# oxfordcontrol/Clarabel.rs

Hardware: NVIDIA H100
Metric: ipm_iterations_per_sec (higher is better)
Workload: dtype f64

## Files before the change

### clarabel.rs_b200/csrc/ldl.cu

```cuda
#include <cuda_runtime.h>
#include <dlfcn.h>

#include <cmath>
#include <cstdio>
#include <cstring>
#include <algorithm>
#include <thread>
#include <vector>

#include "../../include/clarabel_b200.h"
#include "ldl_device.h"
#include "symbolic.h"
#include "vec.cuh"

namespace cb {

std::atomic<unsigned long long> g_launches{0};

typedef struct ncclComm* cb_ncclComm_t;
typedef struct { char internal[128]; } cb_ncclUniqueId;
struct NcclApi {
  void* lib = nullptr;
  int (*GetUniqueId)(cb_ncclUniqueId*) = nullptr;
  int (*CommInitRank)(cb_ncclComm_t*, int, cb_ncclUniqueId, int) = nullptr;
  int (*AllGather)(const void*, void*, size_t, int, cb_ncclComm_t, cudaStream_t) = nullptr;
  int (*CommDestroy)(cb_ncclComm_t) = nullptr;
  const char* (*GetErrorString)(int) = nullptr;
};
static NcclApi* nccl_api(const char* libpath) {
  static NcclApi api;
  static bool tried = false;
  if (api.lib) return &api;
  if (tried && !libpath) return nullptr;
  tried = true;
  void* h = dlopen(libpath && *libpath ? libpath : "libnccl.so.2", RTLD_NOW | RTLD_GLOBAL);
  if (!h) { std::fprintf(stderr, "[clarabel_b200] dlopen(%s) failed: %s\n", libpath ? libpath : "libnccl.so.2", dlerror()); return nullptr; }
  api.GetUniqueId = (int (*)(cb_ncclUniqueId*))dlsym(h, "ncclGetUniqueId");
  api.CommInitRank = (int (*)(cb_ncclComm_t*, int, cb_ncclUniqueId, int))dlsym(h, "ncclCommInitRank");
  api.AllGather = (int (*)(const void*, void*, size_t, int, cb_ncclComm_t, cudaStream_t))dlsym(h, "ncclAllGather");
  api.CommDestroy = (int (*)(cb_ncclComm_t))dlsym(h, "ncclCommDestroy");
  api.GetErrorString = (const char* (*)(int))dlsym(h, "ncclGetErrorString");
  if (!api.GetUniqueId || !api.CommInitRank || !api.AllGather || !api.CommDestroy) return nullptr;
  api.lib = h;
  return &api;
}



template <int NT>
__device__ __forceinline__ void pivot_inverse(double* A, int lda, int ns) {
  for (int j = threadIdx.x; j < ns; j += NT) {
    for (int i = j + 1; i < ns; i++) {
      double a0 = A[(long long)j * lda + i], a1 = 0.0;
      int k = j + 1;
      for (; k + 1 < i; k += 2) {
        a0 += A[(long long)k * lda + i] * A[(long long)k * lda + j];
        a1 += A[(long long)(k + 1) * lda + i] * A[(long long)(k + 1) * lda + j];
      }
      if (k < i) a0 += A[(long long)k * lda + i] * A[(long long)k * lda + j];
      A[(long long)i * lda + j] = -(a0 + a1);
    }
  }
}
template <int NT>
__device__ __forceinline__ void pivot_inverse_place(double* A, int lda, int ns) {
  for (int idx = threadIdx.x; idx < ns * ns; idx += NT) {
    const int j = idx / ns, i = idx - j * ns;
    if (i > j) {
      A[(long long)j * lda + i] = A[(long long)i * lda + j];
      A[(long long)i * lda + j] = 0.0;
    }
  }
}

template <int NT>
__global__ void __launch_bounds__(NT) k_factor_level(LDLDev d, int task_base, int smem_cap) {
  extern __shared__ double sm[];
  __shared__ double sD[CB_MAX_PANEL];
  __shared__ double sInv[CB_MAX_PANEL];
  const int tid = threadIdx.x;
  const int lane = tid & 31, warp = tid >> 5, nwarp = NT >> 5;
  const int s = d.level_tasks[task_base + blockIdx.x];
  const int f = d.sn_first[s];
  const int ns = d.sn_first[s + 1] - f;
  const long long rp = d.sn_rowptr[s];
  const int nr = (int)(d.sn_rowptr[s + 1] - rp);
  const int ld = ns + nr;
  double* __restrict__ P = d.L + d.panel_off[s];
  double* __restrict__ U = d.U + d.upd_off[s];
  const long long psz = (long long)ld * ns;
  const bool use_sm = psz <= (long long)smem_cap;
  double* W = use_sm ? sm : P;

  for (long long i = tid; i < psz; i += NT) W[i] = 0.0;
  __syncthreads();
  for (long long e = d.asm_ptr[s] + tid; e < d.asm_ptr[s + 1]; e += NT)
    W[d.asm_dst[e]] = d.vals[d.asm_src[e]];

  int c_reg = 0, c_pos = 0, c_zero = 0, c_nonf = 0;
  for (int j = 0; j < ns; j++) {
    __syncthreads();
    const double* __restrict__ cj = W + (long long)j * ld;
    double dj = cj[j];
    bool reg = false;
    if (d.reg_enable) {
      const double sg = (double)d.dsigns[f + j];
      if (dj * sg < d.reg_eps) { dj = d.reg_delta * sg; reg = true; }
    }
    const double inv = 1.0 / dj;
    if (tid == 0) {
      c_reg += reg ? 1 : 0;
      c_pos += dj > 0.0 ? 1 : 0;
      if (dj == 0.0) c_zero = 1;
      if (!isfinite(inv)) c_nonf = 1;
      d.D[f + j] = dj;
      d.Dinv[f + j] = inv;
      sD[j] = dj;
      sInv[j] = inv;
    }
    for (int k = j + 1 + warp; k < ns; k += nwarp) {
      const double wk = cj[k] * inv;
      double* __restrict__ ck = W + (long long)k * ld;
      for (int i = k + lane; i < ld; i += 32) ck[i] -= cj[i] * wk;
    }
  }
  __syncthreads();
  for (int j = warp; j < ns; j += nwarp) {
    double* __restrict__ cj = W + (long long)j * ld;
    const double inv = sInv[j];
    if (lane == 0) cj[j] = sD[j];
    for (int i = j + 1 + lane; i < ld; i += 32) cj[i] *= inv;
  }
  if (tid == 0) {
    if (c_reg) atomicAdd(&d.status[ST_REGCOUNT], c_reg);
    if (c_pos) atomicAdd(&d.status[ST_POSINERTIA], c_pos);
    if (c_zero) atomicExch(&d.status[ST_ZEROPIV], 1);
    if (c_nonf) atomicExch(&d.status[ST_NONFINITE], 1);
  }
  __syncthreads();

  {
    int it = 0;
    for (int b0 = 0; b0 < nr; b0 += 4)
      for (int a0 = b0; a0 < nr; a0 += 32, it++) {
        if (it % nwarp != warp) continue;
        const int a = a0 + lane;
        const bool on = a < nr;
        const int nb = min(4, nr - b0);
        double acc[4] = {0.0, 0.0, 0.0, 0.0};
        const double* __restrict__ ck = W + ns;
        for (int k = 0; k < ns; k++, ck += ld) {
          const double la = on ? ck[a] : 0.0, dk = sD[k];
#pragma unroll
          for (int c = 0; c < 4; c++) acc[c] += la * (ck[b0 + min(c, nb - 1)] * dk);
        }
#pragma unroll
        for (int c = 0; c < 4; c++)
          if (on && b0 + c < nr && a >= b0 + c) U[(long long)(b0 + c) * nr + a] = 0.0 - acc[c];
      }
  }
  if (ns > CB_SOLVE_SMALL_NS) {
    pivot_inverse<NT>(W, ld, ns);
    __syncthreads();
    pivot_inverse_place<NT>(W, ld, ns);
  }
  if (use_sm) {
    __syncthreads();
    for (long long i = tid; i < psz; i += NT) P[i] = W[i];
  }
}

#define LEAF1_NT 256
#define LEAF1_MAXLD 128
static_assert(LEAF1_MAXLD > CB_BIG_NR, "a level-0 column must fit the per-warp buffer");
__global__ void __launch_bounds__(LEAF1_NT) k_factor_leaf1(LDLDev d, int task_base, int count) {
  __shared__ double s_col[LEAF1_NT / 32][LEAF1_MAXLD];
  __shared__ int s_pos, s_reg;
  const int lane = threadIdx.x & 31, warp = threadIdx.x >> 5;
  const int i = blockIdx.x * (LEAF1_NT / 32) + warp;
  if (threadIdx.x == 0) { s_pos = 0; s_reg = 0; }
  __syncthreads();
  if (i < count) {
    double* col = s_col[warp];
    const int s = d.level_tasks[task_base + i];
    const int f = d.sn_first[s];
    const long long rp = d.sn_rowptr[s];
    const int nr = (int)(d.sn_rowptr[s + 1] - rp);
    const int ld = 1 + nr;
    double* __restrict__ P = d.L + d.panel_off[s];
    double* __restrict__ U = d.U + d.upd_off[s];
    for (int a = lane; a < ld; a += 32) col[a] = 0.0;
    __syncwarp();
    for (long long e = d.asm_ptr[s] + lane; e < d.asm_ptr[s + 1]; e += 32) col[d.asm_dst[e]] = d.vals[d.asm_src[e]];
    __syncwarp();
    double dj = col[0];
    bool reg = false;
    if (d.reg_enable) {
      const double sg = (double)d.dsigns[f];
      if (dj * sg < d.reg_eps) { dj = d.reg_delta * sg; reg = true; }
    }
    const double inv = 1.0 / dj;
    if (lane == 0) {
      if (dj == 0.0) atomicExch(&d.status[ST_ZEROPIV], 1);
      if (!isfinite(inv)) atomicExch(&d.status[ST_NONFINITE], 1);
      if (dj > 0.0) atomicAdd(&s_pos, 1);
      if (reg) atomicAdd(&s_reg, 1);
      d.D[f] = dj;
      d.Dinv[f] = inv;
    }
    __syncwarp();
    for (int a = lane; a < ld; a += 32) {
      const double v = a == 0 ? dj : col[a] * inv;
      col[a] = v;
      P[a] = v;
    }
    __syncwarp();
    for (int idx = lane; idx < nr * nr; idx += 32) {
      const int b = idx / nr, a = idx - b * nr;
      if (a >= b) {
        const double t = col[1 + b] * dj;
        double acc = 0.0;
        acc += col[1 + a] * t;
        U[idx] = 0.0 - acc;
      }
    }
  }
  __syncthreads();
  if (threadIdx.x == 0) {
    if (s_pos) atomicAdd(&d.status[ST_POSINERTIA], s_pos);
    if (s_reg) atomicAdd(&d.status[ST_REGCOUNT], s_reg);
  }
}

__global__ void k_permute_in(int n, const int* __restrict__ perm, const double* __restrict__ b,
                             double* __restrict__ xp) {
  int k = blockIdx.x * blockDim.x + threadIdx.x;
  if (k < n) xp[k] = b[perm[k]];
}

__device__ __forceinline__ unsigned long long df_gtime() {
#ifdef CB_EMU
  return 0;
#else
  unsigned long long t;
  asm volatile("mov.u64 %0, %%globaltimer;" : "=l"(t));
  return t;
#endif
}
__device__ __forceinline__ void df_wait_zero(volatile int* p) {
  unsigned ns = 20;
  while (*p > 0) { __nanosleep(ns); if (ns < 640) ns <<= 1; }
}
__device__ __forceinline__ void df_wait_set(volatile int* p) {
  unsigned ns = 20;
  while (*p == 0) { __nanosleep(ns); if (ns < 640) ns <<= 1; }
}

#include "ldl_solve.cuh"

#define DF_NT 256
#define DF_SMEM_DOUBLES (CB_PB_MAXNS * CB_PB_LD + 2 * CB_PB_MAXNS + CB_PB_MAXNS * 128)

__device__ __forceinline__ double ldcg_d(const double* p) { return __ldcg(p); }

template <class Map>
__device__ __forceinline__ void df_apply_sorted(double* base, const double* __restrict__ U,
                                                const int* __restrict__ esrc, const int* __restrict__ edst,
                                                int e0, int e1, Map map) {
  const int cnt = e1 - e0;
  if (cnt <= 0) return;
  const int per = (cnt + DF_NT - 1) / DF_NT;
  int b = e0 + threadIdx.x * per, e = min(e1, b + per);
  if (b >= e1) return;
  if (b > e0) { while (b < e1 && edst[b] == edst[b - 1]) b++; }
  if (e < e1) { while (e < e1 && edst[e] == edst[e - 1]) e++; }
  int i = b;
  while (i < e) {
    const int dd = edst[i];
    double acc = 0.0;
    while (i < e && edst[i] == dd) { acc += __ldcg(U + esrc[i]); i++; }
    const long long t = map(dd);
    if (t >= 0) base[t] += acc;
  }
}

__shared__ int df_cur_qi;
#define DF_STAMP(q, slot) do { if ((q).trace && threadIdx.x == 0) (q).trace[10 * (size_t)df_cur_qi + (slot)] = df_gtime(); } while (0)
__device__ __forceinline__ void df_front_complete(const DFFactor& q, int s) {
  const int p = q.parent[s];
  if (p >= 0) atomicSub(q.pend + p, 1);
}

__device__ void dff_small(const LDLDev& d, int s, double* sm, int* s_flag) {
  __shared__ double s_inv;
  const int tid = threadIdx.x, lane = tid & 31, warp = tid >> 5, nwarp = DF_NT >> 5;
  const int f = d.sn_first[s];
  const int ns = d.sn_first[s + 1] - f;
  const long long rp = d.sn_rowptr[s];
  const int nr = (int)(d.sn_rowptr[s + 1] - rp);
  const int ld = ns + nr;
  double* P = d.L + d.panel_off[s];
  double* U = d.U + d.upd_off[s];
  const long long psz = (long long)ld * ns;
  double* sD = sm;
  double* Wsm = sm + CB_MAX_PANEL;
  const bool use_sm = psz <= (long long)(DF_SMEM_DOUBLES - CB_MAX_PANEL);
  double* W = use_sm ? Wsm : P;
  (void)s_flag;
  for (long long i = tid; i < psz; i += DF_NT) W[i] = 0.0;
  for (int b = warp; b < nr; b += nwarp)
    for (int a = b + lane; a < nr; a += 32) U[(long long)b * nr + a] = 0.0;
  __syncthreads();
  for (long long e = d.asm_ptr[s] + tid; e < d.asm_ptr[s + 1]; e += DF_NT) W[d.asm_dst[e]] = d.vals[d.asm_src[e]];
  __syncthreads();
  for (long long ci = d.child_ptr[s]; ci < d.child_ptr[s + 1]; ci++) {
    const int c = d.child_list[ci];
    const long long crp = d.sn_rowptr[c];
    const int nrc = (int)(d.sn_rowptr[c + 1] - crp);
    const double* Uc = d.U + d.upd_off[c];
    const int* __restrict__ relc = d.rel + crp;
    for (int b = warp; b < nrc; b += nwarp) {
      const int rb = relc[b];
      for (int a = b + lane; a < nrc; a += 32) {
        const int ra = relc[a];
        const double v = __ldcg(Uc + (long long)b * nrc + a);
        if (rb < ns) W[(long long)rb * ld + ra] += v;
        else U[(long long)(rb - ns) * nr + (ra - ns)] += v;
      }
    }
    __syncthreads();
  }
  int c_reg = 0, c_pos = 0, c_zero = 0, c_nonf = 0;
  for (int j = 0; j < ns; j++) {
    if (tid == 0) {
      double dj = W[(long long)j * ld + j];
      if (d.reg_enable) {
        const double sg = (double)d.dsigns[f + j];
        if (dj * sg < d.reg_eps) { dj = d.reg_delta * sg; c_reg++; }
      }
      if (dj == 0.0) c_zero = 1;
      if (dj > 0.0) c_pos++;
      const double inv = 1.0 / dj;
      if (!isfinite(inv)) c_nonf = 1;
      d.D[f + j] = dj;
      d.Dinv[f + j] = inv;
      W[(long long)j * ld + j] = dj;
      s_inv = inv;
      sD[j] = dj;
    }
    __syncthreads();
    const double inv = s_inv;
    const double* cj = W + (long long)j * ld;
    for (int k = j + 1 + warp; k < ns; k += nwarp) {
      const double wk = cj[k] * inv;
      double* ck = W + (long long)k * ld;
      for (int i = k + lane; i < ld; i += 32) ck[i] -= cj[i] * wk;
    }
    __syncthreads();
    double* cjw = W + (long long)j * ld;
    for (int i = j + 1 + tid; i < ld; i += DF_NT) cjw[i] *= inv;
  }
  __syncthreads();
  if (tid == 0) {
    if (c_reg) atomicAdd(&d.status[ST_REGCOUNT], c_reg);
    if (c_pos) atomicAdd(&d.status[ST_POSINERTIA], c_pos);
    if (c_zero) atomicExch(&d.status[ST_ZEROPIV], 1);
    if (c_nonf) atomicExch(&d.status[ST_NONFINITE], 1);
  }
  for (int b = warp; b < nr; b += nwarp)
    for (int a = b + lane; a < nr; a += 32) {
      double acc = 0.0;
      for (int k = 0; k < ns; k++) {
        const double* ck = W + (long long)k * ld + ns;
        acc += ck[a] * (ck[b] * sD[k]);
      }
      U[(long long)b * nr + a] -= acc;
    }
  if (ns > CB_SOLVE_SMALL_NS) {
    pivot_inverse<DF_NT>(W, ld, ns);
    __syncthreads();
    pivot_inverse_place<DF_NT>(W, ld, ns);
    __syncthreads();
  }
  if (use_sm) for (long long i = tid; i < psz; i += DF_NT) P[i] = W[i];
}

#define DF_DCAP 32
#define DF_REC_INTS ((int)(sizeof(DFChildRec) / sizeof(int)))
#define DF_REC_INT(r, field) (reinterpret_cast<const int*>(r)[offsetof(DFChildRec, field) / sizeof(int)])

template <int NH>
__device__ __forceinline__ void df_add_child(const LDLDev& d, const DFChildRec& ch, double* dst, int rowoff,
                                             int rstride, int coloff, int cstride) {
  const int lane = threadIdx.x & 31, warp = threadIdx.x >> 5;
  const int* __restrict__ relc = d.rel + ch.relp;
  const double* Uc = d.U + ch.uoff;
  __syncwarp();
  if (ch.contig == 3) {
    const int r0 = ch.ra0 - rowoff - ch.a0, c0 = ch.rb0 - coloff - ch.b0;
    const int bfirst = ch.b0 + ((warp - (c0 + ch.b0)) & 7);
    const int a1 = ch.a1, b1 = ch.b1;
    for (int ab = ch.a0; ab < a1; ab += 32 * NH) {
      double v[8][NH];
#pragma unroll
      for (int c = 0; c < 8; c++) {
        const int b = bfirst + 8 * c;
#pragma unroll
        for (int h = 0; h < NH; h++) {
          const int a = ab + lane + 32 * h;
          v[c][h] = (b < b1 && a < a1 && a >= b) ? __ldcg(Uc + (long long)b * ch.nrc + a) : 0.0;
        }
      }
#pragma unroll
      for (int c = 0; c < 8; c++) {
        const int b = bfirst + 8 * c;
#pragma unroll
        for (int h = 0; h < NH; h++) {
          const int a = ab + lane + 32 * h;
          if (b < b1 && a < a1 && a >= b) dst[(r0 + a) * rstride + (c0 + b) * cstride] += v[c][h];
        }
      }
    }
    __syncwarp();
    return;
  }
  const int bl = ch.b0 + lane, bh = bl + 32;
  const int dc0 = bl < ch.b1 ? relc[bl] - coloff : -1;
  const int dc1 = bh < ch.b1 ? relc[bh] - coloff : -1;
  unsigned m0 = __ballot_sync(0xffffffffu, dc0 >= 0 && (dc0 & 7) == warp);
  unsigned m1 = __ballot_sync(0xffffffffu, dc1 >= 0 && (dc1 & 7) == warp);
  const int cnt0 = __popc(m0), cnt = cnt0 + __popc(m1);
  const int oc = lane >> 2, ar = lane & 3;
  int pos = -1;
  if (oc < cnt) {
    unsigned m = oc < cnt0 ? m0 : m1;
    const int skip = oc < cnt0 ? oc : oc - cnt0;
    for (int k = 0; k < skip; k++) m &= m - 1;
    pos = __ffs(m) - 1 + (oc < cnt0 ? 0 : 32);
  }
  const int srcl = pos < 0 ? 0 : (pos & 31);
  const int x0 = __shfl_sync(0xffffffffu, dc0, srcl), x1 = __shfl_sync(0xffffffffu, dc1, srcl);
  if (pos >= 0) {
    const int dcc = (pos < 32 ? x0 : x1) * cstride;
    const int b = ch.b0 + pos;
    const double* ucol = Uc + (long long)b * ch.nrc;
    const int a1 = ch.a1;
    for (int a = max(ch.a0, b) + ar; a < a1; a += 32) {
      double v[8];
      int r[8];
#pragma unroll
      for (int u = 0; u < 8; u++) {
        const int aa = a + 4 * u;
        const bool ok = aa < a1;
        v[u] = ok ? __ldcg(ucol + aa) : 0.0;
        r[u] = ok ? relc[aa] : rowoff;
      }
#pragma unroll
      for (int u = 0; u < 8; u++)
        if (a + 4 * u < a1) dst[(r[u] - rowoff) * rstride + dcc] += v[u];
    }
  }
  __syncwarp();
}

#define DF_ENT_FAST (2 * DF_NT)
struct DFEnt { int dd[2]; double v[2]; };
__device__ __forceinline__ void df_ent_issue(const double* __restrict__ U, const int* __restrict__ esrc,
                                             const int* __restrict__ edst, int e0, int e1, DFEnt& pe) {
  const int cnt = e1 - e0;
  pe.dd[0] = pe.dd[1] = -1;
  pe.v[0] = pe.v[1] = 0.0;
  if (cnt > DF_ENT_FAST) return;
  int src[2] = {0, 0};
#pragma unroll
  for (int u = 0; u < 2; u++) {
    const int i = threadIdx.x + u * DF_NT;
    if (i < cnt) { pe.dd[u] = edst[e0 + i]; src[u] = esrc[e0 + i]; }
  }
#pragma unroll
  for (int u = 0; u < 2; u++)
    if (threadIdx.x + u * DF_NT < cnt) pe.v[u] = __ldcg(U + src[u]);
}
template <class Map>
__device__ __forceinline__ void df_ent_apply(double* base, const double* __restrict__ U, const int* __restrict__ esrc,
                                             const int* __restrict__ edst, int e0, int e1, const DFEnt& pe,
                                             int* s_ed, double* s_ev, Map map) {
  const int cnt = e1 - e0;
  if (cnt <= 0) return;
  if (cnt > DF_ENT_FAST) { df_apply_sorted(base, U, esrc, edst, e0, e1, map); return; }
#pragma unroll
  for (int u = 0; u < 2; u++) {
    const int i = threadIdx.x + u * DF_NT;
    if (i < cnt) { s_ed[i] = pe.dd[u]; s_ev[i] = pe.v[u]; }
  }
  __syncthreads();
#pragma unroll
  for (int u = 0; u < 2; u++) {
    int i = threadIdx.x + u * DF_NT;
    if (i < cnt) {
      const int dd = pe.dd[u];
      if (i == 0 || s_ed[i - 1] != dd) {
        double acc = 0.0;
        while (i < cnt && s_ed[i] == dd) { acc += s_ev[i]; i++; }
        const long long t = map(dd);
        if (t >= 0) base[t] += acc;
      }
    }
  }
}

template <class Put>
__device__ __forceinline__ void df_scatter_asm(const LDLDev& d, int s, Put put) {
  const long long e0 = d.asm_ptr[s], e1 = d.asm_ptr[s + 1];
  for (long long e = e0 + threadIdx.x; e < e1; e += 4 * DF_NT) {
    long long dst[4];
    int src[4];
    double v[4];
#pragma unroll
    for (int u = 0; u < 4; u++) {
      const long long ee = e + (long long)u * DF_NT;
      const bool ok = ee < e1;
      dst[u] = ok ? (long long)d.asm_dst[ee] : -1;
      src[u] = ok ? d.asm_src[ee] : 0;
    }
#pragma unroll
    for (int u = 0; u < 4; u++) v[u] = dst[u] >= 0 ? d.vals[src[u]] : 0.0;
#pragma unroll
    for (int u = 0; u < 4; u++) if (dst[u] >= 0) put(dst[u], v[u]);
  }
}

template <class F>
__device__ __forceinline__ void df_children(const DFFactor& q, int d0, int d1, int* s_desc, F f) {
  for (int base = d0; base < d1; base += DF_DCAP) {
    const int cnt = min(DF_DCAP, d1 - base);
    const int* src = reinterpret_cast<const int*>(q.recs);
    for (int i = threadIdx.x; i < cnt * DF_REC_INTS; i += DF_NT) s_desc[i] = src[(size_t)base * DF_REC_INTS + i];
// ... 230 lines not shown
  DF_STAMP(q, 6);
#ifdef CB_EMU
  const int tx = tid & 15, ty = tid >> 4;
#define OWN_R(i) (tx + 16 * (i))
#define OWN_C(j) (ty + 16 * (j))
#else
  const int lk = tid & 3, lr = (tid & 31) >> 2, r0w = ((tid >> 5) & 1) * 32, c0w = (tid >> 6) * 16;
#define OWN_R(i) (r0w + 8 * (i) + lr)
#define OWN_C(j) (c0w + 8 * ((j) >> 1) + 2 * lk + ((j) & 1))
#endif
  double creg[4][4];
#pragma unroll
  for (int i = 0; i < 4; i++)
#pragma unroll
    for (int j = 0; j < 4; j++) creg[i][j] = 0.0;
  const int ndense = tk.ndense;
  for (int kd = 0; kd < ndense; kd++) {
    const DFChildRec* rec = q.recs + (size_t)(tk.d0 + kd);
    const long long uoff = rec->uoff;
    const int nrc = DF_REC_INT(rec, nrc), a0 = DF_REC_INT(rec, a0), a1 = DF_REC_INT(rec, a1), b0 = DF_REC_INT(rec, b0), b1 = DF_REC_INT(rec, b1);
    const int ra = a0 - (DF_REC_INT(rec, ra0) - (ns + i0)), rb = b0 - (DF_REC_INT(rec, rb0) - (ns + j0));
    const double* Uc = d.U + uoff;
    double v[4][4];
#pragma unroll
    for (int j = 0; j < 4; j++) {
      const int b = OWN_C(j) + rb;
#pragma unroll
      for (int i = 0; i < 4; i++) {
        const int a = OWN_R(i) + ra;
        v[i][j] = (a >= a0 && a < a1 && b >= b0 && b < b1 && a >= b) ? __ldcg(Uc + (long long)b * nrc + a) : 0.0;
      }
    }
#pragma unroll
    for (int i = 0; i < 4; i++)
#pragma unroll
      for (int j = 0; j < 4; j++) creg[i][j] += v[i][j];
  }
  const bool use_sc = (tk.d1 - tk.d0 > ndense) || (tk.e1 > tk.e0);
  if (use_sc) {
    for (int idx = tid; idx < TS * (TS + 1); idx += DF_NT) sC[idx] = 0.0;
    __syncthreads();
    DF_STAMP(q, 7);
    df_children(q, tk.d0 + ndense, tk.d1, s_desc, [&](const DFChildRec& ch) { df_add_child<2>(d, ch, sC, ns + i0, TS + 1, ns + j0, 1); });
    DF_STAMP(q, 8);
    df_ent_apply(sC, d.U, d.sc_tile_src, d.sc_tile_dst, tk.e0, tk.e1, pe, s_ed, s_ev, [&](int dd) -> long long { return dd; });
  }
#ifndef CB_EMU
  asm volatile("cp.async.wait_group 0;" ::: "memory");
#endif
  __syncthreads();
  for (int idx = tid; idx < ns * TS; idx += DF_NT) sBt[idx] *= sD[idx >> 6];
#ifndef CB_EMU
  {
    const int ns4 = (ns + 3) & ~3;
    for (int idx = ns * TS + tid; idx < ns4 * TS; idx += DF_NT) { sAt[idx] = 0.0; sBt[idx] = 0.0; }
  }
#endif
  __syncthreads();
  DF_STAMP(q, 4);
#ifdef CB_EMU
  double acc[4][4];
#pragma unroll
  for (int i = 0; i < 4; i++)
#pragma unroll
    for (int j = 0; j < 4; j++) acc[i][j] = 0.0;
#pragma unroll 4
  for (int k = 0; k < ns; k++) {
    double a[4], b[4];
#pragma unroll
    for (int i = 0; i < 4; i++) { a[i] = sAt[k * TS + tx + 16 * i]; b[i] = sBt[k * TS + ty + 16 * i]; }
#pragma unroll
    for (int i = 0; i < 4; i++)
#pragma unroll
      for (int j = 0; j < 4; j++) acc[i][j] += a[i] * b[j];
  }
#else
  double c2[4][2][2];
  {
#pragma unroll
    for (int i = 0; i < 4; i++)
#pragma unroll
      for (int j = 0; j < 2; j++) { c2[i][j][0] = 0.0; c2[i][j][1] = 0.0; }
    const int ns4 = (ns + 3) & ~3;
#pragma unroll 2
    for (int k = 0; k < ns4; k += 4) {
      double a[4], b[2];
#pragma unroll
      for (int i = 0; i < 4; i++) a[i] = sAt[(k + lk) * TS + r0w + 8 * i + lr];
#pragma unroll
      for (int j = 0; j < 2; j++) b[j] = sBt[(k + lk) * TS + c0w + 8 * j + lr];
#pragma unroll
      for (int i = 0; i < 4; i++)
#pragma unroll
        for (int j = 0; j < 2; j++)
          asm volatile("mma.sync.aligned.m8n8k4.row.col.f64.f64.f64.f64 {%0,%1}, {%2}, {%3}, {%0,%1};"
                       : "+d"(c2[i][j][0]), "+d"(c2[i][j][1]) : "d"(a[i]), "d"(b[j]));
    }
  }
#endif
  DF_STAMP(q, 5);
#pragma unroll
  for (int i = 0; i < 4; i++) {
    const int rr = OWN_R(i);
#pragma unroll
    for (int j = 0; j < 4; j++) {
      const int cc = OWN_C(j);
#ifdef CB_EMU
      const double prod = acc[i][j];
#else
      const double prod = c2[i][j >> 1][j & 1];
#endif
      if (rr < ni && cc < nj && (i0 + rr >= j0 + cc))
        U[(long long)(j0 + cc) * nr + (i0 + rr)] = (use_sc ? creg[i][j] + sC[rr * (TS + 1) + cc] : creg[i][j]) - prod;
    }
  }
#undef OWN_R
#undef OWN_C
}

__global__ void __launch_bounds__(DF_NT, 2) k_factor_df(LDLDev d, DFFactor q) {
  extern __shared__ __align__(16) double dfsm[];
  __shared__ __align__(16) int s_desc[DF_DCAP * DF_REC_INTS];
  __shared__ __align__(16) int s_task[16];
  __shared__ int s_ed[DF_ENT_FAST];
  __shared__ double s_ev[DF_ENT_FAST];
  __shared__ int s_last;
  const int tid = threadIdx.x;
  if (tid == 0) df_cur_qi = -1;
  for (;;) {
    __syncthreads();
    if (tid == 0) {
      if (q.trace && df_cur_qi >= 0) q.trace[10 * (size_t)df_cur_qi + 2] = df_gtime();
      const int qi = atomicAdd(q.qhead, 1);
      df_cur_qi = qi < q.ntask ? qi : -1;
      if (q.trace && df_cur_qi >= 0) {
        unsigned smid = 0;
#ifndef CB_EMU
        asm volatile("mov.u32 %0, %%smid;" : "=r"(smid));
#endif
        q.trace[10 * (size_t)qi] = df_gtime();
        q.trace[10 * (size_t)qi + 3] = smid;
      }
    }
    __syncthreads();
    const int qi = df_cur_qi;
    if (qi < 0) break;
    if (tid < 4) reinterpret_cast<int4*>(s_task)[tid] = q.tasks[4 * (size_t)qi + tid];
    __syncthreads();
    const DFTask& tk = *reinterpret_cast<const DFTask*>(s_task);
    const int kind = tk.kind, s = tk.s;
    if (kind == 0) {
      if (tid == 0) { df_wait_zero(q.pend + s); __threadfence(); if (q.trace) q.trace[10 * (size_t)qi + 1] = df_gtime(); }
      __syncthreads();
      dff_small(d, s, dfsm, nullptr);
      __syncthreads();
      if (tid == 0) { __threadfence(); df_front_complete(q, s); }
    } else if (kind == 1) {
      if (tid == 0) { df_wait_zero(q.pend + s); __threadfence(); if (q.trace) q.trace[10 * (size_t)qi + 1] = df_gtime(); }
      __syncthreads();
      dff_diag(d, q, tk, dfsm, s_desc, s_ed, s_ev);
      __syncthreads();
      if (tid == 0) { __threadfence(); atomicExch(q.diag_done + s, 1); }
    } else if (kind == 2) {
      if (tid == 0) { df_wait_zero(q.pend + s); __threadfence(); if (q.trace) q.trace[10 * (size_t)qi + 1] = df_gtime(); }
      __syncthreads();
      dff_rows(d, q, tk, dfsm, s_desc, s_ed, s_ev);
      __syncthreads();
      if (tid == 0) { __threadfence(); s_last = atomicSub(q.rows_left + s, 1) == 1; }
      __syncthreads();
      if (s_last && tk.ns > CB_SOLVE_SMALL_NS) dff_rows_invert(d, tk, dfsm);
    } else {
      if (tid == 0) { df_wait_zero(q.rows_left + s); __threadfence(); if (q.trace) q.trace[10 * (size_t)qi + 1] = df_gtime(); }
      __syncthreads();
      dff_tile(d, q, tk, dfsm, s_desc, s_ed, s_ev);
      __syncthreads();
      if (tid == 0) {
        __threadfence();
        if (atomicSub(q.tiles_left + s, 1) == 1) df_front_complete(q, s);
      }
    }
  }
}

__global__ void k_update_values(double* __restrict__ vals, const int* __restrict__ idx,
                                const double* __restrict__ v, long long len) {
  long long i = (long long)blockIdx.x * blockDim.x + threadIdx.x;
  if (i < len) vals[idx[i]] = v[i];
}
__global__ void k_scale_values(double* __restrict__ vals, const int* __restrict__ idx, double s,
                               long long len) {
  long long i = (long long)blockIdx.x * blockDim.x + threadIdx.x;
  if (i < len) vals[idx[i]] *= s;
}
__global__ void k_offset_values(double* __restrict__ vals, const int* __restrict__ idx, double off,
                                const signed char* __restrict__ sg, long long len) {
  long long i = (long long)blockIdx.x * blockDim.x + threadIdx.x;
  if (i < len) {
    const int s = sg[i];
    if (s > 0) vals[idx[i]] += off;
    else if (s < 0) vals[idx[i]] -= off;
  }
}


#define CK(x)                                                                        \
  do {                                                                               \
    cudaError_t e_ = (x);                                                            \
    if (e_ != cudaSuccess) {                                                         \
      std::fprintf(stderr, "[clarabel_b200] CUDA error %s at %s:%d\n",              \
                   cudaGetErrorString(e_), __FILE__, __LINE__);                      \
      return CLDL_E_CUDA;                                                            \
    }                                                                                \
  } while (0)

int LDLObject::init(int n_, const int64_t* Ap, const int32_t* Ai, const double* Ax,
                    const int8_t* dsigns, const cldl_opts& o, const int* perm_in) {
  n = n_;
  opts = o;
  int ndev = 0;
  if (cudaGetDeviceCount(&ndev) != cudaSuccess || ndev == 0) {
    std::fprintf(stderr, "[clarabel_b200] no CUDA device: this backend has no CPU fallback\n");
    return CLDL_E_CUDA;
  }
  device = o.device;
  CK(cudaSetDevice(device));
  SymbolicOptions so;
  so.ordering = o.ordering ? o.ordering : ORDER_BEST;
  so.amd_dense_scale = o.amd_dense_scale > 0 ? o.amd_dense_scale : 1.5;
  if (o.max_panel > 0) so.max_panel = o.max_panel > CB_PB_MAXNS ? CB_PB_MAXNS : o.max_panel;
  if (o.nd_leaf > 0) so.nd_leaf = o.nd_leaf;
  cb_tmark(nullptr);
  int rc = analyse(n, Ap, Ai, perm_in, so, S);
  cb_tmark("ldl: ordering + symbolic");
  if (rc == -2) return CLDL_E_EMPTY_COLUMN;
  if (rc == -3) return CLDL_E_NOT_TRIU;
  if (rc == -5) return CLDL_E_BAD_PERM;
  if (rc) return CLDL_E_ARG;
  shard_nranks = o.shard_nranks > 1 ? o.shard_nranks : 1;
  shard_rank = o.shard_rank;
  if (sharded()) {
    if (shard_rank < 0 || shard_rank >= shard_nranks) return CLDL_E_ARG;
    std::vector<int> par(S.sn_parent);
    if (plan_shards(S.nsup, S.sn_first.data(), S.sn_rowptr.data(), par.data(), shard_nranks, shard)) return CLDL_E_ARG;
    shard_cut.assign(shard_nranks, {});
    shard_xidx.assign(shard_nranks, {});
    for (int s = 0; s < S.nsup; s++) {
      const int g = shard.owner[s];
      if (g < 0) continue;
      if (S.sn_parent[s] >= 0 && shard.owner[S.sn_parent[s]] < 0) shard_cut[g].push_back(s);
      for (int j = S.sn_first[s]; j < S.sn_first[s + 1]; j++) shard_xidx[g].push_back(S.perm[j]);
    }
  }

  CK(cudaStreamCreateWithFlags(&stream, cudaStreamNonBlocking));
  CK(cudaStreamCreateWithFlags(&stream_a, cudaStreamNonBlocking));
  CK(cudaStreamCreateWithFlags(&stream_b, cudaStreamNonBlocking));
  for (auto& e : ev_leaf) CK(cudaEventCreateWithFlags(&e, cudaEventDisableTiming));
  CK(cudaEventCreate(&ev0));
  CK(cudaEventCreate(&ev1));
  CK(cudaMallocHost((void**)&h_status, ST_COUNT * sizeof(int)));

  auto to_ll = [](const std::vector<int64_t>& v) { return std::vector<long long>(v.begin(), v.end()); };
  CK(upload(&dev.sn_first, S.sn_first));
  CK(upload(&dev.sn_rowptr, to_ll(S.sn_rowptr)));
  CK(upload(&dev.sn_rows, S.sn_rows));
  CK(upload(&dev.child_ptr, to_ll(S.child_ptr)));
  CK(upload(&dev.child_list, S.child_list));
  CK(upload(&dev.rel, S.rel));
  CK(upload(&dev.panel_off, to_ll(S.panel_off)));
  CK(upload(&dev.upd_off, to_ll(S.upd_off)));
  CK(upload(&dev.asm_ptr, to_ll(S.asm_ptr)));
  CK(upload(&dev.asm_src, S.asm_src));
  CK(upload(&dev.asm_dst, to_ll(S.asm_dst)));
  CK(upload(&dev.perm, S.perm));
  {
    std::vector<signed char> ds(n);
    for (int k = 0; k < n; k++) ds[k] = dsigns ? (signed char)dsigns[S.perm[k]] : (signed char)1;
    CK(upload(&dev.dsigns, ds));
  }
  nnzA = Ap[n];
  CK(cudaMalloc((void**)&dev.vals, (size_t)(nnzA ? nnzA : 1) * sizeof(double)));
  CK(cudaMemcpy(dev.vals, Ax, (size_t)nnzA * sizeof(double), cudaMemcpyHostToDevice));
  big_alloc_rc = 0;
  big_alloc = std::thread([this]() {
    if (cudaSetDevice(device) != cudaSuccess) { big_alloc_rc = 1; return; }
    const size_t nu = S.sn_rows.size() ? S.sn_rows.size() : 1;
    if (cudaMalloc((void**)&dev.L, ((size_t)(S.L_alloc ? S.L_alloc : 1) + 8) * sizeof(double)) != cudaSuccess ||
        cudaMalloc((void**)&dev.U, (size_t)(S.upd_total ? S.upd_total : 1) * sizeof(double)) != cudaSuccess ||
        cudaMalloc((void**)&dev.u, nu * sizeof(double)) != cudaSuccess ||
        cudaMalloc((void**)&d_u2, nu * sizeof(double)) != cudaSuccess)
      big_alloc_rc = 1;
  });
  struct BigJoin { std::thread& t; ~BigJoin() { if (t.joinable()) t.join(); } } big_join{big_alloc};
  CK(cudaMalloc((void**)&dev.D, (size_t)n * sizeof(double)));
  CK(cudaMalloc((void**)&dev.Dinv, (size_t)n * sizeof(double)));
  CK(cudaMalloc((void**)&d_xp, (size_t)n * sizeof(double)));
  CK(cudaMalloc((void**)&d_xp2, (size_t)n * sizeof(double)));
  CK(cudaMalloc((void**)&d_bx, (size_t)2 * n * sizeof(double)));
  CK(cudaMalloc((void**)&dev.status, ST_COUNT * sizeof(int)));
  CK(cudaMemset(dev.status, 0, ST_COUNT * sizeof(int)));
  dev.reg_enable = o.regularize_enable;
  dev.reg_eps = o.regularize_eps;
  dev.reg_delta = o.regularize_delta;

  cb_tmark("ldl: uploads + device alloc");
  int max_optin = 0, nsm = 0;
  CK(cudaDeviceGetAttribute(&max_optin, cudaDevAttrMaxSharedMemoryPerBlockOptin, device));
// ... 721 lines not shown
```

Before: 26.06.

## Parallelize pivot inverse across warps and share front factor code with dataflow path

```diff
diff --git a/clarabel.rs_b200/csrc/ldl.cu b/clarabel.rs_b200/csrc/ldl.cu
--- a/clarabel.rs_b200/csrc/ldl.cu
+++ b/clarabel.rs_b200/csrc/ldl.cu
@@ -47,18 +47,49 @@
 
 
 
+#define PINV_CW 4
 template <int NT>
 __device__ __forceinline__ void pivot_inverse(double* A, int lda, int ns) {
-  for (int j = threadIdx.x; j < ns; j += NT) {
-    for (int i = j + 1; i < ns; i++) {
-      double a0 = A[(long long)j * lda + i], a1 = 0.0;
-      int k = j + 1;
-      for (; k + 1 < i; k += 2) {
-        a0 += A[(long long)k * lda + i] * A[(long long)k * lda + j];
-        a1 += A[(long long)(k + 1) * lda + i] * A[(long long)(k + 1) * lda + j];
+  constexpr int nwarp = NT / 32, RP = 2;
+  static_assert(CB_PB_MAXNS == 32 * RP, "a lane owns two rows of the pivot block");
+  const int lane = threadIdx.x & 31, warp = threadIdx.x >> 5;
+  const int ngroup = (ns - 1 + PINV_CW - 1) / PINV_CW;
+  for (int p = 0; p * nwarp < ngroup; p++) {
+    const int g = p * nwarp + ((p & 1) ? nwarp - 1 - warp : warp);
+    if (g >= ngroup) continue;
+    const int j0 = g * PINV_CW;
+    double a0[RP][PINV_CW], a1[RP][PINV_CW];
+#pragma unroll
+    for (int r = 0; r < RP; r++)
+#pragma unroll
+      for (int c = 0; c < PINV_CW; c++) {
+        const int i = lane + 32 * r;
+        a0[r][c] = (i > j0 + c && i < ns) ? A[(long long)(j0 + c) * lda + i] : 0.0;
+        a1[r][c] = 0.0;
       }
-      if (k < i) a0 += A[(long long)k * lda + i] * A[(long long)k * lda + j];
-      A[(long long)i * lda + j] = -(a0 + a1);
+#pragma unroll 1
+    for (int k = j0 + 1; k < ns; k++) {
+      double* colk = A + (long long)k * lda;
+      double l[RP];
+#pragma unroll
+      for (int r = 0; r < RP; r++) {
+        const int i = lane + 32 * r;
+        l[r] = (i > k && i < ns) ? colk[i] : 0.0;
+      }
+#pragma unroll
+      for (int c = 0; c < PINV_CW; c++) {
+        const int j = j0 + c;
+        if (j < k) {
+          const double v = k < 32 ? -(a0[0][c] + a1[0][c]) : -(a0[1][c] + a1[1][c]);
+          const double x = __shfl_sync(0xffffffffu, v, k & 31);
+          if (lane == (k & 31)) colk[j] = x;
+#pragma unroll
+          for (int r = 0; r < RP; r++) {
+            if ((k - j) & 1) a0[r][c] = fma(l[r], x, a0[r][c]);
+            else a1[r][c] = fma(l[r], x, a1[r][c]);
+          }
+        }
+      }
     }
   }
 }
@@ -73,30 +104,13 @@
   }
 }
 
-template <int NT>
-__global__ void __launch_bounds__(NT) k_factor_level(LDLDev d, int task_base, int smem_cap) {
-  extern __shared__ double sm[];
-  __shared__ double sD[CB_MAX_PANEL];
-  __shared__ double sInv[CB_MAX_PANEL];
+template <int NT, bool ACCUM>
+__device__ __forceinline__ void front_factor(const LDLDev& d, int f, int ns, int nr, double* W, double* __restrict__ P,
+                                             double* __restrict__ U, bool use_sm, double* sD, double* sInv) {
   const int tid = threadIdx.x;
   const int lane = tid & 31, warp = tid >> 5, nwarp = NT >> 5;
-  const int s = d.level_tasks[task_base + blockIdx.x];
-  const int f = d.sn_first[s];
-  const int ns = d.sn_first[s + 1] - f;
-  const long long rp = d.sn_rowptr[s];
-  const int nr = (int)(d.sn_rowptr[s + 1] - rp);
   const int ld = ns + nr;
-  double* __restrict__ P = d.L + d.panel_off[s];
-  double* __restrict__ U = d.U + d.upd_off[s];
   const long long psz = (long long)ld * ns;
-  const bool use_sm = psz <= (long long)smem_cap;
-  double* W = use_sm ? sm : P;
-
-  for (long long i = tid; i < psz; i += NT) W[i] = 0.0;
-  __syncthreads();
-  for (long long e = d.asm_ptr[s] + tid; e < d.asm_ptr[s + 1]; e += NT)
-    W[d.asm_dst[e]] = d.vals[d.asm_src[e]];
-
   int c_reg = 0, c_pos = 0, c_zero = 0, c_nonf = 0;
   for (int j = 0; j < ns; j++) {
     __syncthreads();
@@ -149,6 +163,7 @@
         const int nb = min(4, nr - b0);
         double acc[4] = {0.0, 0.0, 0.0, 0.0};
         const double* __restrict__ ck = W + ns;
+#pragma unroll 1
         for (int k = 0; k < ns; k++, ck += ld) {
           const double la = on ? ck[a] : 0.0, dk = sD[k];
 #pragma unroll
@@ -156,7 +171,10 @@
         }
 #pragma unroll
         for (int c = 0; c < 4; c++)
-          if (on && b0 + c < nr && a >= b0 + c) U[(long long)(b0 + c) * nr + a] = 0.0 - acc[c];
+          if (on && b0 + c < nr && a >= b0 + c) {
+            double* u = U + (long long)(b0 + c) * nr + a;
+            *u = (ACCUM ? *u : 0.0) - acc[c];
+          }
       }
   }
   if (ns > CB_SOLVE_SMALL_NS) {
@@ -168,6 +186,28 @@
     __syncthreads();
     for (long long i = tid; i < psz; i += NT) P[i] = W[i];
   }
+}
+
+template <int NT>
+__global__ void __launch_bounds__(NT, 1024 / NT) k_factor_level(LDLDev d, int task_base, int smem_cap) {
+  extern __shared__ double sm[];
+  __shared__ double sD[CB_MAX_PANEL];
+  __shared__ double sInv[CB_MAX_PANEL];
+  const int tid = threadIdx.x;
+  const int s = d.level_tasks[task_base + blockIdx.x];
+  const int f = d.sn_first[s];
+  const int ns = d.sn_first[s + 1] - f;
+  const int nr = (int)(d.sn_rowptr[s + 1] - d.sn_rowptr[s]);
+  double* __restrict__ P = d.L + d.panel_off[s];
+  const long long psz = (long long)(ns + nr) * ns;
+  const bool use_sm = psz <= (long long)smem_cap;
+  double* W = use_sm ? sm : P;
+
+  for (long long i = tid; i < psz; i += NT) W[i] = 0.0;
+  __syncthreads();
+  for (long long e = d.asm_ptr[s] + tid; e < d.asm_ptr[s + 1]; e += NT)
+    W[d.asm_dst[e]] = d.vals[d.asm_src[e]];
+  front_factor<NT, false>(d, f, ns, nr, W, P, d.U + d.upd_off[s], use_sm, sD, sInv);
 }
 
 #define LEAF1_NT 256
@@ -291,8 +331,7 @@
   if (p >= 0) atomicSub(q.pend + p, 1);
 }
 
-__device__ void dff_small(const LDLDev& d, int s, double* sm, int* s_flag) {
-  __shared__ double s_inv;
+__device__ void dff_small(const LDLDev& d, int s, double* sm) {
   const int tid = threadIdx.x, lane = tid & 31, warp = tid >> 5, nwarp = DF_NT >> 5;
   const int f = d.sn_first[s];
   const int ns = d.sn_first[s + 1] - f;
@@ -303,10 +342,10 @@
   double* U = d.U + d.upd_off[s];
   const long long psz = (long long)ld * ns;
   double* sD = sm;
-  double* Wsm = sm + CB_MAX_PANEL;
-  const bool use_sm = psz <= (long long)(DF_SMEM_DOUBLES - CB_MAX_PANEL);
+  double* sInv = sm + CB_MAX_PANEL;
+  double* Wsm = sm + 2 * CB_MAX_PANEL;
+  const bool use_sm = psz <= (long long)(DF_SMEM_DOUBLES - 2 * CB_MAX_PANEL);
   double* W = use_sm ? Wsm : P;
-  (void)s_flag;
   for (long long i = tid; i < psz; i += DF_NT) W[i] = 0.0;
   for (int b = warp; b < nr; b += nwarp)
     for (int a = b + lane; a < nr; a += 32) U[(long long)b * nr + a] = 0.0;
@@ -330,59 +369,7 @@
     }
     __syncthreads();
   }
-  int c_reg = 0, c_pos = 0, c_zero = 0, c_nonf = 0;
-  for (int j = 0; j < ns; j++) {
-    if (tid == 0) {
-      double dj = W[(long long)j * ld + j];
-      if (d.reg_enable) {
-        const double sg = (double)d.dsigns[f + j];
-        if (dj * sg < d.reg_eps) { dj = d.reg_delta * sg; c_reg++; }
-      }
-      if (dj == 0.0) c_zero = 1;
-      if (dj > 0.0) c_pos++;
-      const double inv = 1.0 / dj;
-      if (!isfinite(inv)) c_nonf = 1;
-      d.D[f + j] = dj;
-      d.Dinv[f + j] = inv;
-      W[(long long)j * ld + j] = dj;
-      s_inv = inv;
-      sD[j] = dj;
-    }
-    __syncthreads();
-    const double inv = s_inv;
-    const double* cj = W + (long long)j * ld;
-    for (int k = j + 1 + warp; k < ns; k += nwarp) {
-      const double wk = cj[k] * inv;
-      double* ck = W + (long long)k * ld;
-      for (int i = k + lane; i < ld; i += 32) ck[i] -= cj[i] * wk;
-    }
-    __syncthreads();
-    double* cjw = W + (long long)j * ld;
-    for (int i = j + 1 + tid; i < ld; i += DF_NT) cjw[i] *= inv;
-  }
-  __syncthreads();
-  if (tid == 0) {
-    if (c_reg) atomicAdd(&d.status[ST_REGCOUNT], c_reg);
-    if (c_pos) atomicAdd(&d.status[ST_POSINERTIA], c_pos);
-    if (c_zero) atomicExch(&d.status[ST_ZEROPIV], 1);
-    if (c_nonf) atomicExch(&d.status[ST_NONFINITE], 1);
-  }
-  for (int b = warp; b < nr; b += nwarp)
-    for (int a = b + lane; a < nr; a += 32) {
-      double acc = 0.0;
-      for (int k = 0; k < ns; k++) {
-        const double* ck = W + (long long)k * ld + ns;
-        acc += ck[a] * (ck[b] * sD[k]);
-      }
-      U[(long long)b * nr + a] -= acc;
-    }
-  if (ns > CB_SOLVE_SMALL_NS) {
-    pivot_inverse<DF_NT>(W, ld, ns);
-    __syncthreads();
-    pivot_inverse_place<DF_NT>(W, ld, ns);
-    __syncthreads();
-  }
-  if (use_sm) for (long long i = tid; i < psz; i += DF_NT) P[i] = W[i];
+  front_factor<DF_NT, true>(d, f, ns, nr, W, P, U, use_sm, sD, sInv);
 }
 
 #define DF_DCAP 32
@@ -919,7 +906,7 @@
     if (kind == 0) {
       if (tid == 0) { df_wait_zero(q.pend + s); __threadfence(); if (q.trace) q.trace[10 * (size_t)qi + 1] = df_gtime(); }
       __syncthreads();
-      dff_small(d, s, dfsm, nullptr);
+      dff_small(d, s, dfsm);
       __syncthreads();
       if (tid == 0) { __threadfence(); df_front_complete(q, s); }
     } else if (kind == 1) {
```

New measurement: 26.52, median of 6. 1.8% higher.
